# poke1024/vectorian

Hardware: AMD Instinct MI355X
Metric: sentence-alignments/sec at d=300, |q|=10, |s|<=64; 1/2/4/8 GPU + %HBM roofline (higher is better)
Workload: dtype bf16

## Files before the change

### vectorian_amd/csrc/vk_bound_host.h

```cpp
#ifndef VK_BOUND_HOST_H
#define VK_BOUND_HOST_H

#include "../../include/vectorian_hip.h"

#include <cmath>
#include <cstdint>
#include <cstring>
#include <vector>

#ifdef __HIPCC__
#define VK_HOST_DEVICE __host__ __device__
#define VK_UNROLL _Pragma("unroll")
#else
#define VK_HOST_DEVICE
#define VK_UNROLL
#endif

namespace vk_host {

struct shadow_format {
	int bits = 0;
	int d = 0;
	int steps = 0, step_features = 0;
	int live = 0, kept = 0;
// ... 132 lines not shown
		uint8_t *xq = codes.data();
		quant_meta m;
		if (fmt.bits == 8) { m = quantize_row_i8(x, d, reinterpret_cast<int8_t *>(xq)); i8_put_row(t.data(), i, xq, d); }
		else { m = quantize_row_e2m3(x, d, xq); fp6_put_row(t.data(), 4, i, xq, d); }
		bound_cell_constants(m, N, X, fmt.gamma_width, &cst[i], &cst[16 + i], &cst[32 + i]);
	}
	out.swap(t);
	return true;
}

struct bound_backoff {
	uint32_t recent = 0;
	int skip = 0;
	bool take() {
		if (skip > 0) { skip--; return false; }
		return true;
	}
	void record(bool fell_back) {
		recent = ((recent << 1) | (fell_back ? 1u : 0u)) & 0xffu;
		if (fell_back && __builtin_popcount(recent) >= 5) { skip = 64; recent = 0; }
	}
};

}

#endif
```

### vectorian_amd/csrc/vk_common.hip.h

```cpp

#ifndef VK_COMMON_HIP_H
#define VK_COMMON_HIP_H

#include <hip/hip_runtime.h>
#include <stdint.h>
#include <stdlib.h>

#include "vk_device.h"

typedef __attribute__((ext_vector_type(8))) short bf16x8;
typedef __attribute__((ext_vector_type(4))) short bf16x4;
typedef __attribute__((ext_vector_type(4))) float f32x4;
typedef __attribute__((ext_vector_type(4))) int i32x4;
typedef __attribute__((ext_vector_type(2))) float f32x2;

#define VK_NEG_INF (-__builtin_inff())
#define VK_RUN 4
#ifdef VK_DBG_NOINLINE
#define VK_DP_INLINE __attribute__((noinline))
#else
#define VK_DP_INLINE __forceinline__
#endif


// ... 186 lines not shown
	}
	return acc;
}
__device__ __forceinline__ f32x4 dot_tile_fp6(const uint8_t *__restrict__ qlds, const uint8_t *__restrict__ tile, int lane, int live6) {
	i32x4 lo[VK_DEV_FP6_STEPS];
	i32x2 hi[VK_DEV_FP6_STEPS];
	f32x2 meta;
	const uint32_t o16 = fp6_lane_offset(lane);
	load_tile_fp6<false>(lo, hi, meta, tile, lane, live6, o16);
	return mma_tile_fp6(lo, hi, qlds, o16);
}

__device__ __forceinline__ f32x4 cell_tile_fp6(const f32x4 acc, const f32x2 m, const uint8_t *__restrict__ qlds, int lane) {
	const float *cst = reinterpret_cast<const float *>(qlds + VK_DEV_FP6_QTILE_BYTES) + (lane >> 4) * 4;
	const f32x4 cs = *reinterpret_cast<const f32x4 *>(cst), ca = *reinterpret_cast<const f32x4 *>(cst + 16), cb = *reinterpret_cast<const f32x4 *>(cst + 32);
	f32x4 ub;
#pragma unroll
	for (int r = 0; r < 4; r++) ub[r] = clip01(((m[0] * cs[r]) * acc[r] + m[1] * ca[r]) + cb[r]);
	return ub;
}

#ifndef VK_FP6_TILES
#define VK_FP6_TILES 2
#endif
template <int T>
__device__ __forceinline__ void sim_tiles_fp6(f32x4 (&ub)[T], const uint8_t *__restrict__ qlds, const uint8_t *__restrict__ tile, int tile_bytes, int lane, int live6) {
	i32x4 lo[T][VK_DEV_FP6_STEPS];
	i32x2 hi[T][VK_DEV_FP6_STEPS];
	f32x2 meta[T];
	const uint32_t o16 = fp6_lane_offset(lane);
#pragma unroll
	for (int i = 0; i < T; i++) load_tile_fp6<true>(lo[i], hi[i], meta[i], tile + (int64_t)i * tile_bytes, lane, live6, o16);
	if constexpr (T > 1) __builtin_amdgcn_sched_barrier(0);
#pragma unroll
	for (int i = 0; i < T; i++) {
		ub[i] = cell_tile_fp6(mma_tile_fp6(lo[i], hi[i], qlds, o16), meta[i], qlds, lane);
		asm volatile("" : "+v"(ub[i]));
	}
}

template <int NB16>
__device__ __forceinline__ f32x4 sim_tile_f32_qlds(const uint8_t *__restrict__ qlds, const uint8_t *__restrict__ tile, int lane) {
	f32x4 x[NB16];
#pragma unroll
	for (int b = 0; b < NB16; b++) x[b] = __builtin_nontemporal_load(reinterpret_cast<const f32x4 *>(tile + b * 1024 + lane * 16));
	__builtin_amdgcn_sched_barrier(0);
// ... 503 lines not shown
			if (LT > 6) hc = fmaxf(hc, dpp_zero<0x116>(c) - wtv[6]);
			if (LT > 7) hc = fmaxf(hc, dpp_zero<0x117>(c) - wtv[7]);
			if (LT > 8) hc = fmaxf(hc, dpp_zero<0x118>(c) - wtv[8]);
			if (LT > 9) hc = fmaxf(hc, dpp_zero<0x119>(c) - wtv[9]);
			if (LT > 10) hc = fmaxf(hc, dpp_zero<0x11a>(c) - wtv[10]);
			if (LT > 11) hc = fmaxf(hc, dpp_zero<0x11b>(c) - wtv[11]);
			if (LT > 12) hc = fmaxf(hc, dpp_zero<0x11c>(c) - wtv[12]);
			if (LT > 13) hc = fmaxf(hc, dpp_zero<0x11d>(c) - wtv[13]);
			if (LT > 14) hc = fmaxf(hc, dpp_zero<0x11e>(c) - wtv[14]);
			if (LT > 15) hc = fmaxf(hc, dpp_zero<0x11f>(c) - wtv[15]);
			hreg[u] = hc;
			h = act ? hc : h;
			if (is_local || last_col) best = fmaxf(best, h);
		}
	}
	float m;
	if (is_local) m = v < a.len_t ? best : 0.0f;
	else if (is_global) m = last_col ? h : VK_NEG_INF;
	else m = v < a.len_t ? fmaxf(h, last_col ? best : 0.0f) : 0.0f;
	m = row_max_to_lane15(m);
	return (is_global) ? m : fmaxf(m, 0.0f);
}

template <int LT>
__device__ __forceinline__ float rwmd_rows(const float *__restrict__ S, int rowbase, int len, int maxlen, int v, const DpArgs &a) {
	const int len_t = a.len_t;
	const bool nbow = a.rwmd_normalize_bow != 0;
	const float w_t = nbow ? 1.0f / (float)len_t : 1.0f;
	const float w_s = nbow ? 1.0f / (float)(len > 0 ? len : 1) : 1.0f;
	const bool col_ok = v < len_t;
	float colmin = 3.402823466e+38F;
	float acc1 = 0.0f;
	for (int u = 1; u <= maxlen; u++) {
		const bool act = u <= len;
		const float s = S[(rowbase + (act ? u - 1 : 0)) * LT + v];
		const float dist = fmaxf(1.0f - s, 0.0f);
		if (act) colmin = fminf(colmin, dist);
		float m = col_ok ? dist : 3.402823466e+38F;
		m = fminf(m, dpp_f<DPP_ROW_SHR1>(m, m));
		m = fminf(m, dpp_f<DPP_ROW_SHR2>(m, m));
		m = fminf(m, dpp_f<DPP_ROW_SHR4>(m, m));
		m = fminf(m, dpp_f<DPP_ROW_SHR8>(m, m));
		if (act) acc1 += w_s * m;
	}
	const float x = col_ok ? w_t * colmin : 0.0f;
	float sum = x;
// ... 175 lines not shown
```

### vectorian_amd/csrc/vk_corpus.cpp

```cpp

#include "vk_internal.h"

std::string &vk_error_slot() {
	static thread_local std::string err;
	return err;
}

std::mutex &vk_ring_mutex() {
	static std::mutex mu;
	return mu;
}

void vk_devblock::release(void *p) {
	if (!p) return;
	{
		std::lock_guard<std::mutex> g(mu);
		ptrs.erase(std::remove(ptrs.begin(), ptrs.end(), p), ptrs.end());
	}
	(void)hipFree(p);
}

vk_devblock::~vk_devblock() {
	(void)hipSetDevice(device);
	for (void *p : ptrs) if (p) (void)hipFree(p);
// ... 540 lines not shown
int vk_bound_pass_state(vk_corpus_t *c, float *bounds, int64_t n, int64_t *counters) {
	if (!c || !counters) return fail(VK_ERR_INVALID, "null argument");
	const int64_t v[7] = {c->bp.ran, c->bp.round1, c->bp.round2, c->bp.fell_back, c->bp.queries, c->bp.fallbacks, c->bp.survivors};
	memcpy(counters, v, sizeof v);
	if (!bounds) return VK_OK;
	if (!c->bp.ran) return fail(VK_ERR_STATE, "the last query ran no bound pass");
	if (n != c->desc.n_sentences) return fail(VK_ERR_INVALID, "n differs from n_sentences");
	VK_HIP(hipSetDevice(c->device));
	std::vector<float> rows((size_t)c->n_entries);
	VK_HIP(hipMemcpy(rows.data(), c->d_ub, rows.size() * 4, hipMemcpyDeviceToHost));
	for (int64_t e = 0; e < c->n_entries; e++) {
		const int64_t sent = c->entry_sent.empty() ? e : (int64_t)c->entry_sent[(size_t)e];
		if (sent >= 0) bounds[sent] = rows[(size_t)e];
	}
	return VK_OK;
}

int vk_bound_pass_bits(vk_corpus_t *c, int64_t *bits) {
	if (!c || !bits) return fail(VK_ERR_INVALID, "null argument");
	*bits = c->shadow ? c->shadow_format.bits : 0;
	return VK_OK;
}

int vk_bound_pass_shadow(vk_corpus_t *c, int64_t *format, float *nx, int64_t tile0, int64_t n, uint8_t *out) {
	if (!c || !format || !nx) return fail(VK_ERR_INVALID, "null argument");
	const vk_host::shadow_format &sf = c->shadow_format;
	const int64_t f[5] = {sf.bits, sf.steps, sf.live, sf.tile_bytes(), c->n_tiles};
	memset(format, 0, sizeof f);
	nx[0] = nx[1] = 0.0f;
	if (!c->shadow) return out ? fail(VK_ERR_STATE, "the corpus has no shadow") : VK_OK;
	memcpy(format, f, sizeof f);
	nx[0] = c->shadow_n; nx[1] = c->shadow_x;
	if (!out) return VK_OK;
	if (tile0 < 0 || n < 0 || tile0 > c->n_tiles || n > c->n_tiles - tile0) return fail(VK_ERR_INVALID, "tiles out of range");
	VK_HIP(hipSetDevice(c->device));
	VK_HIP(hipStreamSynchronize(c->stream));
	if (n > 0) VK_HIP(hipMemcpy(out, c->shadow + tile0 * sf.tile_bytes(), (size_t)n * sf.tile_bytes(), hipMemcpyDeviceToHost));
	return VK_OK;
}

int vk_batch_state(vk_corpus_t *c, int64_t *state) {
	if (!c || !state) return fail(VK_ERR_INVALID, "null argument");
	memcpy(state, c->batch_state, sizeof c->batch_state);
	return VK_OK;
}

// ... 65 lines not shown
```

### vectorian_amd/csrc/vk_device.h

```cpp
#ifndef VK_DEVICE_H
#define VK_DEVICE_H

#include <hip/hip_runtime.h>
#include <stdint.h>

#define VK_DEV_LOCAL 0
#define VK_DEV_GLOBAL 1
#define VK_DEV_SEMIGLOBAL 2

#define VK_DEV_LAYOUT_CONTEXTUAL 0
#define VK_DEV_LAYOUT_STATIC 1

#define VK_DEV_MAX_SENT_LEN 64
#define VK_DEV_MAX_LONG_LEN 512
#define VK_DEV_MAX_QUERY_LEN 16
#define VK_DEV_MAX_WIDE_QUERY_LEN 64
#define VK_DEV_BOUND_CONST_BYTES 256
#define VK_DEV_FP6_STEPS 3
#define VK_DEV_FP6_STEP_BYTES 1536
#define VK_DEV_FP6_QTILE_BYTES (VK_DEV_FP6_STEPS * VK_DEV_FP6_STEP_BYTES)
#define VK_DEV_FP6_TILE_BYTES(live6) ((VK_DEV_FP6_STEPS - 1) * VK_DEV_FP6_STEP_BYTES + 384 * (live6) + 128)

struct VkScoreParams {
	const uint8_t *tiles;
	const int32_t *tok_id;
	const float *table;
	const int32_t *sent_start;
	const int32_t *sent_end;
	int32_t n_sent;
	int32_t layout;
	int32_t nk32, tail, tile_bytes;
	int32_t prec;
	int32_t q_lds;
	int32_t bound_bits;
	int32_t bound_live;
	int32_t q_mode3;
	const int32_t *group_list;
	int32_t n_list;
	int32_t max_short_len;
	const uint8_t *qtile;
	int32_t len_t;
	int32_t locality;
	int32_t gap_mode;
	int32_t rwmd_symmetric, rwmd_normalize_bow;
// ... 4 lines not shown
	const float *ws;
	const float *wt;
	const float *wt0;
	const float *boost;
	const int8_t *pos_s;
	const int8_t *tag_s;
	const uint32_t *qid_bits;
	int32_t slices_overlap;
	int32_t qkey[VK_DEV_MAX_QUERY_LEN];
	float tw[VK_DEV_MAX_QUERY_LEN];
	int32_t tpos[VK_DEV_MAX_QUERY_LEN];
	float tw_keep;
	float tw_threshold;
	float ref_total;
	const float *mag;
	float qmass[VK_DEV_MAX_QUERY_LEN];
	float wrd_raw_total;
	float *scores;
	float *raw;
	int32_t lds_floats_per_wave;
	int32_t s_rows_per_wave;
	int32_t h_rows;
	int32_t m_rows;
};

struct VkRwmdBatchParams {
	const uint8_t *tiles;
	int64_t n_tiles;
	int32_t tile_bytes, nk, half;
	const uint8_t *qtiles;
	int32_t n_qtiles, qpt;
	int32_t dense;
	int32_t late_mask;
	const int32_t *q_len;
	const float *q_inv_len;
	const float *q_param;
	int32_t n_queries;
	int32_t n_sent;
	int32_t tiles_per_sent;
	int32_t symmetric, nbow;
	const float *boost;
	float *scores;
	const int32_t *sent_len;
	const int32_t *sent_id;
	int64_t score_stride;
	const int32_t *tok_id;
// ... 236 lines not shown
hipError_t vk_launch_i8_probe(const int8_t *q, const int8_t *x, int32_t *out, hipStream_t stream);
hipError_t vk_launch_fp6_bound_probe(const uint8_t *qtile6, const uint8_t *tile6, int32_t live6, float *out, hipStream_t stream);
hipError_t vk_launch_select_ge_key(const float *scores, int64_t n, const uint64_t *theta_key, float floor_excl, uint64_t *keys_out,
	uint32_t *counter, uint32_t cap, hipStream_t stream);
hipError_t vk_launch_rekey(const uint64_t *keys, int32_t n, const float *scores, float floor_excl, uint64_t *out, hipStream_t stream);
hipError_t vk_launch_topk_unsorted(const uint64_t *in, int32_t n, int32_t k, uint64_t *out, hipStream_t stream);
hipError_t vk_launch_key_groups(const uint64_t *keys, int32_t n, int32_t *groups, hipStream_t stream);
hipError_t vk_launch_pack(const void *in, int32_t dtype_bf16, int64_t n_rows, int32_t d, int32_t d_pad, int64_t row0,
	uint8_t *tiles, float *mag_out, int32_t normalize, int32_t prec, hipStream_t stream);
size_t vk_score32_lds_bytes(int32_t nk32, int32_t tail, int32_t max_pair_tiles, int32_t len_t, int32_t gap_mode, int32_t waves);
int32_t vk_score32_waves(int32_t nk32, int32_t tail, int32_t max_pair_tiles, int32_t len_t, int32_t gap_mode);
hipError_t vk_launch_score32(const VkWideParams *p, int32_t max_pair_tiles, hipStream_t stream);
hipError_t vk_launch_filter_scan(const int8_t *pos, const int8_t *tag, uint64_t pos_mask, uint64_t tag_mask, int64_t n,
	int32_t *keep, int32_t *new_index, void *temp, size_t *temp_bytes, hipStream_t stream);
hipError_t vk_launch_filter_maps(const int32_t *keep, const int32_t *new_index, int64_t n, int32_t *src_of,
	const int32_t *start, const int32_t *end, int64_t n_entries, int32_t *out_start, int32_t *out_end, hipStream_t stream);
hipError_t vk_launch_filter_rows(const uint8_t *src, uint8_t *dst, const int32_t *src_of, int64_t n_kept, int32_t tile_bytes,
	hipStream_t stream);
hipError_t vk_launch_filter_gather(const void *src, void *dst, int32_t elem_bytes, const int32_t *src_of, int64_t n_kept,
	hipStream_t stream);
hipError_t vk_launch_table(const uint8_t *etiles, const uint8_t *qtile, int32_t n_tiles, int32_t nk32, int32_t tail,
	int32_t tile_bytes, float *table, const int32_t *q_ids, int32_t len_t, int32_t V, int32_t prec, hipStream_t stream);
hipError_t vk_launch_score(const VkScoreParams *p, int32_t grid, size_t smem_bytes, hipStream_t stream);
hipError_t vk_launch_span(const VkScoreParams *p, hipStream_t stream);
hipError_t vk_launch_score_batch(const VkScoreBatchParams *p, int32_t lt, size_t smem, hipStream_t stream);
hipError_t vk_launch_topk_scores(const float *scores, int64_t n, float min_score, int32_t k, uint64_t *out,
	int32_t *n_blocks_out, hipStream_t stream);
hipError_t vk_launch_topk_keys(const uint64_t *in, int64_t n, int32_t k, uint64_t *out, int32_t *n_blocks_out,
	hipStream_t stream);
hipError_t vk_launch_topk_wave(const float *scores, const uint64_t *keys_in, int64_t n, float min_score, int32_t k,
	int64_t per_wave, uint64_t *out, int64_t *n_waves_out, hipStream_t stream);
hipError_t vk_launch_flow(const VkFlowParams *p, int32_t k, hipStream_t stream);
hipError_t vk_launch_sort_all(const float *scores, int64_t n, float min_score, uint64_t *keys_a, uint64_t *keys_b, void *temp, size_t *temp_bytes,
	uint64_t **sorted_out, hipStream_t stream);
hipError_t vk_launch_rwmd_batch(const VkRwmdBatchParams *p, hipStream_t stream);
hipError_t vk_launch_rwmd_batch32(const VkRwmdBatchParams *p, hipStream_t stream);
hipError_t vk_launch_batch_pack(const uint8_t *src_tiles, uint8_t *dst_tiles, const int32_t *ids, const int32_t *sent_start, const int32_t *sent_end,
	int64_t n, int32_t tps, int32_t tile_bytes, hipStream_t stream);
int vk_rwmd_batch_supported(int32_t nk, int32_t half);
hipError_t vk_launch_table_batch(const uint8_t *etiles, int64_t n_vtiles, int32_t tile_bytes, int32_t nk16, const uint8_t *qtiles, int32_t n_qtiles,
	uint16_t *table, hipStream_t stream);
hipError_t vk_launch_table_batch_fix(uint16_t *table, const int64_t *offsets, int32_t n, hipStream_t stream);
hipError_t vk_launch_rwmd_static32(const VkRwmdBatchParams *p, int32_t w64, hipStream_t stream);
hipError_t vk_launch_topk_wave_batch(const float *scores, const uint64_t *keys_in, int64_t n, float min_score, int32_t k,
	int64_t per_wave, int32_t n_queries, int64_t in_stride, int64_t out_stride, uint64_t *out, int64_t *n_waves_out, hipStream_t stream);
hipError_t vk_launch_wrd_exact(const VkWrdParams *p, int32_t n_cand, float *scores_to_mark, hipStream_t stream);
// ... 13 lines not shown
```

### vectorian_amd/csrc/vk_internal.h

```cpp
#ifndef VK_INTERNAL_H
#define VK_INTERNAL_H

#include "../../include/vectorian_hip.h"
#include "vk_device.h"
#include "vk_devbuf.h"
#include "vk_guard.h"
#include "vk_result_host.h"
#include "vk_bound_host.h"
#include "vk_route_host.h"

#include <algorithm>
#include <atomic>
#include <cmath>
#include <cstdio>
#include <cstring>
#include <memory>
#include <mutex>
#include <string>
#include <vector>

std::string &vk_error_slot();

namespace {

// ... 24 lines not shown
	uint32_t u = ((uint32_t)b) << 16;
	float f;
	memcpy(&f, &u, 4);
	return f;
}

using vk_host::gap_cost;

constexpr int kTopkChunk = 2048;
constexpr int kGapTable = 640;
constexpr int64_t kStageBytes = 64ll << 20;
constexpr int64_t kBoundPassMinSentences = 1000000;
constexpr int64_t kBoundRound2Floor = 1024;
inline int bound_pass_mode() {
	const char *e = getenv("VK_BOUND_PASS");
	return !e ? 0 : !strcmp(e, "off") ? -1 : !strcmp(e, "force") ? 1 : 0;
}
inline int bound_bits_wanted(int mode) {
	const char *e = getenv("VK_BOUND_BITS");
	if (e && !strcmp(e, "6")) return 6;
	if (e && !strcmp(e, "8")) return 8;
	return mode > 0 ? 8 : 6;
}

}

struct vk_devblock {
	int device = 0;
	std::mutex mu;
	std::vector<void *> ptrs;
	void add(void *p) { std::lock_guard<std::mutex> g(mu); ptrs.push_back(p); }
	void release(void *p);
	~vk_devblock();
};

std::mutex &vk_ring_mutex();

struct vk_corpus_shape {
	vk_corpus_desc desc{};
	int device = 0;
	int d_pad = 0, nk32 = 0, tail = 0, tile_bytes = 0;
	int prec = 0;
	int64_t rows_total = 0, rows_appended = 0, n_tiles = 0;
	uint8_t *d_tiles = nullptr;
	float *d_mag = nullptr;
	int32_t *d_tok_id = nullptr;
// ... 54 lines not shown
	vk_devbuf<float> d_out_raw, d_out_sim;
	vk_devbuf<int16_t> d_out_map;
	vk_devbuf<float> d_wrd_raw, d_wrd_val;
	vk_devbuf<uint32_t> d_counter;
	vk_devbuf<float> d_rows_out, d_plan_out;
	vk_devbuf<uint8_t> d_bqt; vk_devbuf<uint64_t> d_bcand; vk_devbuf<int32_t> d_bcandq; vk_devbuf<float> d_brows;
	vk_devbuf<float, true> h_brows;
	vk_devbuf<uint32_t> d_qbits;
	vk_devbuf<uint8_t> d_wrdl_scratch;
	vk_devbuf<uint8_t> d_wide_scratch;
	vk_devbuf<int32_t> d_apart_order; int32_t n_apart_order = -1;
	vk_devbuf<int32_t> d_xlong_order; int32_t n_xlong_order = -1;
	vk_devbuf<int32_t> d_wide_order; int32_t n_wide_order = -1;
	int rows_w = 0;
	struct batch_bucket { vk_devbuf<uint8_t> tiles; vk_devbuf<int32_t> len, id; int64_t n = 0; };
	batch_bucket bl[4];
	bool bl_built = false;
	int64_t bl_empty = 0;
	vk_devbuf<uint8_t> d_qtile8; vk_devbuf<float> d_ub; vk_devbuf<int32_t> d_bound_groups; vk_devbuf<uint64_t> d_bound_keys;
	struct bound_state {
		bool pruned = false;
		VkScoreParams full{}; int full_grid = 0; size_t full_smem = 0;
		int64_t ran = 0, round1 = 0, round2 = 0, fell_back = 0;
		int64_t queries = 0, fallbacks = 0, survivors = 0;
		vk_host::bound_backoff backoff;
	} bp;
	vk_devbuf<int32_t> d_sb_id[2]; int64_t sb_n[2] = {0, 0}; bool sb_built = false; int64_t sb_empty = 0;
	vk_devbuf<uint16_t> d_btable;
	vk_devbuf<int64_t> d_bfix;
	vk_devbuf<int32_t> d_bqids;
	vk_devbuf<uint64_t> d_sort[2]; vk_devbuf<uint8_t> d_sort_temp;
	int64_t batch_state[VK_BS_COUNT] = {};
	int64_t query_route[VK_QR_COUNT] = {};
	hipEvent_t ev[7] = {nullptr, nullptr, nullptr, nullptr, nullptr, nullptr, nullptr};
	vk_timings last{};
	bool have_scores = false;
	bool is_view = false;
	struct longq_bufs {
		vk_devbuf<uint8_t> qt;
		vk_devbuf<float> fl;
		vk_devbuf<int32_t> il;
		vk_devbuf<float> table;
		vk_devbuf<uint8_t> scratch, fscratch;
		vk_devbuf<uint8_t> bscratch;
		vk_devbuf<int32_t> order; int32_t n_order = -1;
		vk_devbuf<float> raw, sim;
// ... 132 lines not shown
```

### vectorian_amd/csrc/vk_query.cpp

```cpp

#include "vk_internal.h"
#include "vk_guard.h"
#include "vk_transport_host.h"

static constexpr int kCanonMargin = 8;
static const vk_host::route_fits kRouteFits{vk_score32_waves, vk_wide_ring_rows, vk_wide_lds_demand};
static bool exact_transport(const vk_query_desc *q) { return vk_host::exact_transport(q->algorithm, q->wmd_full != 0); }
static vk_host::route_facts route_facts_of(const vk_corpus *c, const vk_query_desc *q, const vk_topk_out *out) {
	vk_host::route_facts f;
	f.layout = c->desc.layout; f.prec = c->prec; f.nk32 = c->nk32; f.tail = c->tail;
	f.max_len = c->max_len; f.max_short_len = c->max_short_len; f.n_long_groups = c->n_long_groups;
	f.has_apart = c->h_apart && !c->h_apart->empty(); f.has_xlong = c->h_xlong && !c->h_xlong->empty();
	f.max_pair_tiles = c->max_pair_tiles; f.max_short_pair_tiles = c->max_short_pair_tiles; f.uniform_len = c->uniform_len;
	f.has_pos = c->d_pos != nullptr; f.has_tags = c->d_tag != nullptr; f.n_sentences = c->desc.n_sentences;
	f.algorithm = q->algorithm; f.wmd_full = q->wmd_full != 0; f.rwmd_injective = q->rwmd_injective != 0; f.len_t = q->len_t;
	if (q->algorithm == VK_ALG_ALIGN) {
		f.gaps = vk_host::classify_gaps(q->gap_s, q->gap_t);
		if (f.gaps.gap_mode == 2 && q->gap_s.kind >= VK_GAP_LINEAR && q->gap_s.kind <= VK_GAP_TABLE) f.ws_tail = vk_host::ws_tail_of(q->gap_s, c->max_len);
	}
	f.submatch = q->submatch_weight > 0.0f; f.tagged = q->tag_weights != nullptr; f.has_q_tags = q->q_tags != nullptr; f.has_q_ids = q->q_token_ids != nullptr;
	f.only = q->only_slices != nullptr; f.want_flow = q->want_flow != 0; f.locality = q->locality;
	f.sim_rows = out->sim_rows != nullptr; f.raw_score = out->raw_score != nullptr; f.boost = q->boost != nullptr;
	const int k = q->max_matches;
	const bool restated = (q->want_flow && q->algorithm == VK_ALG_ALIGN) || (q->algorithm == VK_ALG_RWMD && !q->wmd_full && q->want_flow && out->sim_rows);
// ... 119 lines not shown
			if (c->prec) {
				const size_t off = (size_t)(i >> 4) * c->tile_bytes + (size_t)(k >> 4) * 1024 + (size_t)((k & 3) * 16 + (i & 15)) * 16 + (size_t)((k & 15) >> 2) * 4;
				memcpy(&tile[off], &row[(size_t)k], 4);
				continue;
			}
			const uint16_t b = f32_to_bf16(row[(size_t)k]);
			const int t = k >> 5, g = (k & 31) >> 3, j = k & 7;
			const size_t off = (size_t)(i >> 4) * c->tile_bytes + (size_t)t * 1024 + (size_t)(g * 16 + (i & 15)) * 16 + (size_t)j * 2;
			memcpy(&tile[off], &b, 2);
		}
	}
	if (!bound_tile || !c->shadow || c->prec || q->len_t > VK_FAST_QUERY_LEN) return;
	std::vector<float> stored((size_t)q->len_t * d);
	for (int i = 0; i < q->len_t; i++)
		for (int k = 0; k < d; k++) {
			uint16_t b;
			memcpy(&b, &tile[(size_t)(k >> 5) * 1024 + (size_t)(((k & 31) >> 3) * 16 + i) * 16 + (size_t)(k & 7) * 2], 2);
			stored[(size_t)i * d + k] = bf16_to_f32(b);
		}
	vk_host::pack_bound_query(c->shadow_format, stored.data(), q->len_t, c->shadow_n, c->shadow_x, *bound_tile);
}

static int score_bounded(vk_corpus *c, const VkScoreParams &p, int grid, size_t smem, size_t smem_bound, size_t smem_list, int kk, float sel_floor,
	vk_host_keep &keep, hipStream_t st, const uint64_t **d_sel) {
	*d_sel = nullptr;
	const int64_t n = c->n_entries;
	vk_corpus::bound_state &b = c->bp;
	const int64_t most = std::max<int64_t>(n / 16, kBoundRound2Floor);
	const int M = kk <= 32 ? 64 : kk <= 256 ? 512 : VK_MAX_MATCHES;
	int rc;
	if ((rc = c->d_ub.reserve((size_t)n + 8, &c->device_bytes))) return rc;
	if ((rc = c->d_bound_groups.reserve((size_t)std::max<int64_t>(most, kTopkChunk), &c->device_bytes))) return rc;
	if ((rc = c->d_bound_keys.reserve((size_t)2 * kTopkChunk, &c->device_bytes))) return rc;
	if ((rc = c->d_counter.reserve(4, &c->device_bytes))) return rc;
	VkScoreParams pb = p;
	const vk_host::shadow_format &sf = c->shadow_format;
	pb.tiles = c->shadow; pb.nk32 = sf.steps; pb.tail = 0; pb.tile_bytes = sf.tile_bytes(); pb.bound_bits = sf.bits; pb.bound_live = sf.live;
	pb.q_mode3 = 0; pb.q_lds = 0; pb.qtile = c->d_qtile8; pb.scores = c->d_ub; pb.raw = nullptr;
	VK_HIP(vk_launch_score(&pb, grid, smem_bound, st));
	VK_HIP(hipEventRecord(c->ev[2], st));
	c->ev2_recorded = true;
	b.ran = 1; b.queries++;
	VK_HIP(hipMemsetD32Async(static_cast<hipDeviceptr_t>(c->d_scores), (int)0xff800000u, (size_t)n, st));
	if (p.raw) VK_HIP(hipMemsetD32Async(reinterpret_cast<hipDeviceptr_t>(p.raw), (int)0xff800000u, (size_t)n, st));
	VkScoreParams pl = p;
	pl.group_list = c->d_bound_groups;
	const uint64_t *d_first = nullptr;
	if ((rc = select_blocks(c, sel_floor, M, st, &d_first, c->d_ub))) return rc;
	VK_HIP(vk_launch_key_groups(d_first, M, c->d_bound_groups, st));
	pl.n_list = M;
	VK_HIP(vk_launch_score(&pl, M, smem_list, st));
	uint64_t *d_exact = c->d_bound_keys, *d_best = c->d_bound_keys + kTopkChunk;
	VK_HIP(vk_launch_rekey(d_first, M, c->d_scores, sel_floor, d_exact, st));
	VK_HIP(vk_launch_topk_unsorted(d_exact, M, kk, d_best, st));
	VK_HIP(vk_launch_select_ge_key(c->d_ub, n, d_best + (kk - 1), sel_floor, c->d_keys[0], c->d_counter, (uint32_t)most, st));
	uint32_t &count = *keep.array<uint32_t>(1);
	VK_HIP(hipMemcpyAsync(&count, c->d_counter, 4, hipMemcpyDeviceToHost, st));
	VK_HIP(hipStreamSynchronize(st));
	b.round1 = M;
	bool fell = false;
	if ((int64_t)count > most) {
// ... 2 lines not shown
	} else if (count > 0) {
		VK_HIP(vk_launch_key_groups(c->d_keys[0], (int32_t)count, c->d_bound_groups, st));
		pl.n_list = (int32_t)count;
		VK_HIP(vk_launch_score(&pl, (int32_t)count, smem_list, st));
	}
	if (!fell && count <= (uint32_t)kTopkChunk) {
		VK_HIP(vk_launch_rekey(c->d_keys[0], (int32_t)count, c->d_scores, sel_floor, d_exact, st));
		VK_HIP(vk_launch_topk_unsorted(d_exact, (int32_t)count, kk, d_best, st));
		*d_sel = d_best;
	}
	b.round2 = count;
	if (!fell) b.survivors += count;
	b.fell_back = fell ? 1 : 0;
	if (fell) b.fallbacks++;
	if (bound_pass_mode() == 0) b.backoff.record(fell);
	b.pruned = !fell;
	b.full = p; b.full_grid = grid; b.full_smem = smem;
	return VK_OK;
}

static int query_body(vk_corpus_t *c, const vk_query_desc *q, vk_topk_out *out, vk_host_keep &keep) {
	int rc = VK_OK;
	VK_HIP(hipSetDevice(c->device));
	c->bp.pruned = false; c->bp.ran = c->bp.round1 = c->bp.round2 = c->bp.fell_back = 0;
	for (int64_t &x : c->query_route) x = -1;
	if (q->len_t > VK_MAX_QUERY_LEN) return vk_longq_query(c, q, out, keep);
	hipStream_t st = c->stream;
	const int64_t n = c->n_entries;
	const int k = q->max_matches;
	const bool only = q->only_slices != nullptr;
	out->n_out = 0;
	c->have_scores = false;
	if (n == 0) return VK_OK;
	const vk_host::route_switches sw = vk_host::read_route_switches();
	vk_host::route_facts facts = route_facts_of(c, q, out);
	const int bound_mode = bound_pass_mode();
	facts.bound_pass = c->shadow && bound_mode >= 0 && (bound_mode > 0 || c->desc.n_sentences >= kBoundPassMinSentences) && vk_host::bound_pass_takes(facts) &&
		(bound_mode != 0 || c->bp.backoff.take());
	const vk_host::query_route r = vk_host::route_query(facts, sw, kRouteFits);
	if (r.status != VK_OK) return fail(r.status, r.message);
	const int64_t route_state[VK_QR_COUNT] = {r.plan, r.gap_mode, r.wide_gap_mode, r.score32_gap_mode, r.wave_tiles, r.pass[vk_host::CLASS_SHORT],
		r.pass[vk_host::CLASS_MID], r.pass[vk_host::CLASS_XLONG], r.list, r.ring_rows, r.flow, r.ostride, r.raw, r.span_skip_raw};
	memcpy(c->query_route, route_state, sizeof route_state);
	const bool wide_query = q->len_t > VK_FAST_QUERY_LEN;
	const bool xlong = c->max_len > VK_MAX_SENT_LEN;
	const bool wide_family = r.flow != vk_host::FLOW_NARROW;
	auto sentence_of = [c](int64_t row) { return c->entry_sent.empty() ? row : (int64_t)c->entry_sent[(size_t)row]; };
// ... 267 lines not shown
	p.m_rows = (c->max_short_len + 4) / 4 * 4;
	if (p.gap_mode == 7) lds_floats += 4 * p.m_rows;
	p.lds_floats_per_wave = lds_floats;
	size_t smem = (size_t)lds_floats * 4 * 4;
	const bool reg_history = p.gap_mode == 3 || p.gap_mode == 6;
	if (!is_static && c->prec == 0 && c->nk32 == 10 && c->tail == 1)
		p.q_mode3 = sw.qlds ? 1 : sw.qreg ? 0 : (reg_history ? 1 : 0);
	if (!is_static && c->prec == 1 && c->nk32 == 19 && !sw.no_f32_special) p.q_mode3 = 1;
	const size_t qlds = (!is_static && ((c->prec == 0 && c->nk32 == 24 && c->tail == 0) || p.q_mode3)) ? (size_t)c->nk32 * 1024 : 0;
	smem += qlds;
	if (!is_static && qlds == 0 && !(c->prec == 0 && c->nk32 == 10 && c->tail == 1)) {
		const size_t qb = ((size_t)c->tile_bytes + 1023) / 1024 * 1024;
		if (2 * (smem + qb) <= 160 * 1024 && !sw.no_qlds1) { p.q_lds = (int32_t)qb; smem += qb; }
	}
	if (smem > 160 * 1024) return fail(VK_ERR_UNSUPPORTED, "LDS demand exceeds 160 KiB per workgroup");
	const int64_t n_groups = (n + 3) / 4;
	const int grid = (int)std::min<int64_t>((n_groups + 3) / 4, (int64_t)1 << 20);
	bounded = bound_ok;
	if (!bounded && r.plan == vk_host::PLAN_BOUNDED) c->query_route[VK_QR_PLAN] = vk_host::PLAN_FUSED;
	if (bounded) {
		const size_t smem_strips = smem - qlds - (size_t)p.q_lds;
		const size_t smem_bound = smem_strips + (size_t)c->shadow_format.qtile_bytes() + VK_DEV_BOUND_CONST_BYTES;
		const size_t smem_list = (size_t)lds_floats * 4 + qlds + (size_t)p.q_lds;
		if ((rc = score_bounded(c, p, grid, smem, smem_bound, smem_list, kk, sel_floor, keep, st, &d_sel_bounded))) return rc;
	} else if (r.plan != vk_host::PLAN_LISTED) VK_HIP(vk_launch_score(&p, grid, smem, st));
	if (r.pass[vk_host::CLASS_MID] == vk_host::PASS_FUSED_LONG) {
		VkScoreParams pl = p;
		pl.group_list = c->d_long_groups; pl.n_list = c->n_long_groups;
		if (pl.gap_mode == 3 || pl.gap_mode == 6) pl.gap_mode = 2;
		pl.s_rows_per_wave = is_static ? (c->long_group_tokens + 15) / 16 * 16 : c->long_group_tiles * 16;
		pl.h_rows = 0;
		int lf = pl.s_rows_per_wave * lt + 16;
		if (pl.gap_mode == 2) lf += (c->max_long_len + 1) * 16;
		pl.m_rows = 0;
		if (pl.gap_mode == 7) lf += (c->max_long_len + 4) / 4 * 4;
		pl.lds_floats_per_wave = lf;
		const size_t smem_l = (size_t)lf * 4 + qlds + (size_t)pl.q_lds;
		if (smem_l > 160 * 1024) return fail(VK_ERR_UNSUPPORTED, "LDS demand of the long-slice pass exceeds 160 KiB");
		VK_HIP(vk_launch_score(&pl, c->n_long_groups, smem_l, st));
	}
	if (r.wide_pass != vk_host::PASS_NONE && (rc = list_pass())) return rc;
	}

	if (exact_transport(q) && only) {
		const int cnt = q->n_only;
		std::vector<uint64_t> &hk = keep.vec<uint64_t>((size_t)cnt);
		std::vector<int64_t> rows_idx((size_t)cnt);
// ... 461 lines not shown
```

### vectorian_amd/csrc/vk_score.hip.h

```cpp
#ifndef VK_SCORE_HIP_H
#define VK_SCORE_HIP_H

#include <type_traits>
#include "vk_common.hip.h"


#ifdef VK_SCORE_VGPRS
#define VK_SCORE_KERNEL_ATTR __attribute__((amdgpu_num_vgpr(VK_SCORE_VGPRS)))
#else
#define VK_SCORE_KERNEL_ATTR
#endif

template <int MODE, int NK32, bool TAIL, int GAP, int LT>
__global__ __launch_bounds__(256) VK_SCORE_KERNEL_ATTR void vk_score_kernel(VkScoreParams p) {
	extern __shared__ float4 vk_smem4[];
	float *smem = reinterpret_cast<float *>(vk_smem4);
	const int lane = threadIdx.x & 63, wv = threadIdx.x >> 6;
	const int nwaves = blockDim.x >> 6;
	const uint8_t *qlds = reinterpret_cast<const uint8_t *>(smem);
	if constexpr (MODE == 3 || MODE == 4) {
		for (int i = threadIdx.x; i < NK32 * 64; i += blockDim.x)
			vk_smem4[i] = *reinterpret_cast<const float4 *>(p.qtile + i * 16);
		__syncthreads();
		smem += NK32 * 256;
// ... 21 lines not shown
	float *S = smem + wv * p.lds_floats_per_wave;
	float *Hh = S + p.s_rows_per_wave * LT + 16;
	const int sigma = lane >> 4, v = lane & 15;

	QFrag<NK32, TAIL> qf;
	if constexpr (MODE == 0) load_qfrag<NK32, TAIL>(qf, p.qtile, lane);

	DpArgs a;
	a.locality = p.locality; a.len_t = p.len_t;
	a.gs = p.gs; a.gt = p.gt; a.a_s = p.a_s; a.a_t = p.a_t; a.open_s = p.open_s; a.open_t = p.open_t;
	a.ws = p.ws; a.wt = p.wt; a.wt0 = p.wt0;
	a.rwmd_symmetric = p.rwmd_symmetric; a.rwmd_normalize_bow = p.rwmd_normalize_bow; a.wmd_bound = p.wmd_bound;
	a.wrd_raw_total = p.wrd_raw_total;
	const float inv_ref = p.ref_total;
	constexpr bool TAGS = MODE != 7 && MODE != 8;
	float twl[4] = {1.0f, 1.0f, 1.0f, 1.0f};
	int tposl[4] = {0, 0, 0, 0};
	if (TAGS && p.pos_s) {
		const int cbase = (MODE == 2) ? (lane & 3) * 4 : (lane >> 4) * 4;
#pragma unroll
		for (int r = 0; r < 4; r++) { twl[r] = p.tw[cbase + r]; tposl[r] = p.tpos[cbase + r]; }
	}

	constexpr int WSN = GAP == 6 ? 65 : 33;
	float wsr[WSN], wtr[LT];
	if (GAP == 3 || GAP == 6) {
#pragma unroll
		for (int k = 0; k < WSN; k++) wsr[k] = p.ws[k];
#pragma unroll
		for (int k = 0; k < LT; k++) wtr[k] = p.wt[k];
	}

	const int n_groups = p.group_list ? p.n_list : (p.n_sent + 3) >> 2;
	const int run = p.group_list ? 1 : VK_RUN;
	const int n_runs = (n_groups + run - 1) / run;
	for (int ri = blockIdx.x * nwaves + wv; ri < n_runs; ri += gridDim.x * nwaves) {
	int prev_tile = -1, prev_row = 0;
	for (int gg = 0; gg < run; gg++) {
		const int gi = ri * run + gg;
		if (gi >= n_groups) break;
		const int grp = p.group_list ? p.group_list[gi] : gi;
		const int s_idx = grp * 4 + sigma;
		const int i0 = s_idx < p.n_sent ? s_idx : p.n_sent;
		const int t_a = p.sent_start[i0], t_b = p.sent_end[i0];
		const int len = t_b - t_a;
		const int g_a = __builtin_amdgcn_readlane(t_a, 0);
		const int g_b = __builtin_amdgcn_readlane(t_b, 48);
		int maxlen = __builtin_amdgcn_readlane(len, 0);
		maxlen = max(maxlen, __builtin_amdgcn_readlane(len, 16));
		maxlen = max(maxlen, __builtin_amdgcn_readlane(len, 32));
		maxlen = max(maxlen, __builtin_amdgcn_readlane(len, 48));
// ... 27 lines not shown
						}
						if ((lane & 3) * 4 < LT) *reinterpret_cast<float4 *>(S + tk * LT + (lane & 3) * 4) = vq;
					}
				}
			}
			rowbase = t_a - g_a;
		} else {
			const int tile0 = g_a >> 4;
			const int ntiles = ((g_b + 15) >> 4) - tile0;
			const uint8_t *tp = p.tiles + (int64_t)tile0 * p.tile_bytes;
			int ti0 = 0;
			if (ntiles > 0 && tile0 == prev_tile) {
				if (prev_row != 0) {
					float4 keep = {0.0f, 0.0f, 0.0f, 0.0f};
					if (lane < 4 * LT) keep = reinterpret_cast<const float4 *>(S)[prev_row * 4 * LT + lane];
					wave_lds_fence();
					if (lane < 4 * LT) reinterpret_cast<float4 *>(S)[lane] = keep;
				}
				ti0 = 1;
				tp += p.tile_bytes;
			}
			if (ntiles > 0) { prev_tile = tile0 + ntiles - 1; prev_row = ntiles - 1; }
			if constexpr (MODE == 8) {
				constexpr int T = GAP == 6 ? 1 : VK_FP6_TILES;
				const auto tiles = [&](auto tc, int ti) {
					constexpr int N = decltype(tc)::value;
					f32x4 ub[N];
					sim_tiles_fp6<N>(ub, qlds, tp, p.tile_bytes, lane, p.bound_live);
#pragma unroll
					for (int i = 0; i < N; i++)
						if ((lane >> 4) * 4 < LT) *reinterpret_cast<f32x4 *>(S + ((ti + i) * 16 + (lane & 15)) * LT + (lane >> 4) * 4) = ub[i];
					tp += (int64_t)N * p.tile_bytes;
				};
				int ti = ti0;
				for (; ti + T <= ntiles; ti += T) tiles(std::integral_constant<int, T>{}, ti);
				if constexpr (T > 1)
					for (; ti < ntiles; ti++) tiles(std::integral_constant<int, 1>{}, ti);
			} else
			for (int ti = ti0; ti < ntiles; ti++) {
				f32x4 acc;
				if constexpr (MODE == 0) acc = sim_tile<NK32, TAIL>(qf, tp, lane);
				else if constexpr (MODE == 3) acc = sim_tile_qlds<NK32, TAIL>(qlds, tp, lane);
				else if constexpr (MODE == 4) acc = sim_tile_f32_qlds<NK32>(qlds, tp, lane);
				else if constexpr (MODE == 7) acc = sim_tile_i8<NK32>(qlds, tp, lane, p.bound_live);
				else {
					constexpr bool DEEP = MODE == 5 || MODE == 6;
					constexpr int PREC = MODE == 6 ? 1 : 0;
// ... 12 lines not shown
		}
		wave_lds_fence();
		int turns = 1;
		bool rewrite = false;
		if constexpr (MODE == 2 && (GAP == 4 || GAP == 7)) {
			if (p.qid_bits) {
				rewrite = len > 0 && static_vocab_shared(len, p.len_t, p.tok_id + t_a, p.tag_s + t_a, p.qid_bits, p.qkey) != 0;
				if (p.slices_overlap && __builtin_amdgcn_ballot_w64(rewrite) != 0) turns = 4;
				else if (rewrite) static_vocab_fixup<16>(S + rowbase * LT, LT, len, p.len_t, p.tok_id + t_a, p.tag_s + t_a, p.pos_s + t_a, p.table, 0,
					p.qid_bits, p.qkey, p.tw, p.tpos, p.tw_keep, p.tw_threshold, v);
				wave_lds_fence();
			}
		}

		const int lenc = len > 0 ? len : 0;
		const int rb = len > 0 ? rowbase : 0;
		auto evaluate = [&]() -> float {
		float raw;
		if constexpr (GAP == 0) raw = dp_linear<LT>(S, rb, lenc, maxlen, v, a);
		else if constexpr (GAP == 1) raw = dp_affine<LT>(S, rb, lenc, maxlen, v, a);
		else if constexpr (GAP == 2) raw = dp_general<LT>(S, Hh, p.h_rows, rb, lenc, maxlen, lane, a);
		else if constexpr (GAP == 3) raw = dp_general_reg<LT, 32>(S, rb, lenc, maxlen, v, a, wsr, wtr);
		else if constexpr (GAP == 6) raw = dp_general_reg<LT, 64, MODE != 7>(S, rb, lenc, maxlen, v, a, wsr, wtr);
		else if constexpr (GAP == 4) {
			if (a.wmd_bound == 1) raw = wrd_bound_rows<LT>(S, rb, lenc, maxlen, v, a, nullptr, nullptr, 1.0f / (float)a.len_t);
			else raw = rwmd_rows<LT>(S, rb, lenc, maxlen, v, a);
		}
		else if constexpr (GAP == 7) {
			float *sm = nullptr;
			if (MODE == 2) {
				sm = Hh + sigma * p.m_rows;
				const float wsum = p.rwmd_normalize_bow ? (float)(lenc > 0 ? lenc : 1) : 1.0f;
				for (int u = v; u < lenc; u += 16) {
					const int id = p.tok_id[t_a + u];
					int cnt = 0;
					bool first = true;
					for (int i = 0; i < lenc; i++) {
						const bool same = p.tok_id[t_a + i] == id && (!p.tag_s || p.tag_s[t_a + i] == p.tag_s[t_a + u]);
						cnt += same ? 1 : 0;
						first = first && !(same && i < u);
					}
					sm[u] = first ? (float)cnt / wsum : 0.0f;
				}
				wave_lds_fence();
			}
			raw = rwmd_fill_rows<LT>(S, sm, rb, lenc, maxlen, lane, a, p.qmass[v]);
// ... 92 lines not shown
```

### vectorian_amd/csrc/vk_score_m7.hip

```cpp
#define VK_SCORE_VGPRS 120
#include "vk_score.hip.h"

extern "C" hipError_t vk_launch_score_m7w(const VkScoreParams *p, int32_t grid, size_t smem_bytes, hipStream_t stream);
template <int NK64>
static hipError_t launch_m7(const VkScoreParams *p, int32_t grid, size_t smem_bytes, hipStream_t stream) {
	switch (p->gap_mode) {
	case 0: return launch_score_lt<7, NK64, false, 0>(*p, grid, smem_bytes, stream);
	case 1: return launch_score_lt<7, NK64, false, 1>(*p, grid, smem_bytes, stream);
	case 3: return launch_score_lt<7, NK64, false, 3>(*p, grid, smem_bytes, stream);
	case 6: return vk_launch_score_m7w(p, grid, smem_bytes, stream);
	default: return hipErrorInvalidValue;
	}
}
extern "C" hipError_t vk_launch_score_m7(const VkScoreParams *p, int32_t grid, size_t smem_bytes, hipStream_t stream) {
	if (p->bound_live < 1 || p->bound_live > 4) return hipErrorInvalidValue;
	if (p->pos_s) return hipErrorInvalidValue;
	if (p->nk32 == 5) return launch_m7<5>(p, grid, smem_bytes, stream);
	if (p->nk32 == 12) return launch_m7<12>(p, grid, smem_bytes, stream);
	return hipErrorInvalidValue;
}
```

### vectorian_amd/csrc/vk_score_m8.hip

```cpp
#define VK_SCORE_VGPRS 120
#include "vk_score.hip.h"

extern "C" hipError_t vk_launch_score_m8w(const VkScoreParams *p, int32_t grid, size_t smem_bytes, hipStream_t stream);
extern "C" hipError_t vk_launch_score_m8(const VkScoreParams *p, int32_t grid, size_t smem_bytes, hipStream_t stream) {
	if (p->bound_live < 1 || p->bound_live > 4 || p->tile_bytes != VK_DEV_FP6_TILE_BYTES(p->bound_live)) return hipErrorInvalidValue;
	if (p->pos_s) return hipErrorInvalidValue;
	switch (p->gap_mode) {
	case 0: return launch_score_lt<8, VK_DEV_FP6_STEPS, false, 0>(*p, grid, smem_bytes, stream);
	case 1: return launch_score_lt<8, VK_DEV_FP6_STEPS, false, 1>(*p, grid, smem_bytes, stream);
	case 3: return launch_score_lt<8, VK_DEV_FP6_STEPS, false, 3>(*p, grid, smem_bytes, stream);
	case 6: return vk_launch_score_m8w(p, grid, smem_bytes, stream);
	default: return hipErrorInvalidValue;
	}
}
```

Before: 720.8 million.

## Use flat-tailed gap table in bound pass to cut DP inner loop cost

Adds a bound-pass DP variant (gap modes 8/9) that keeps only the first K gap costs exactly and replaces all longer gaps with the minimum tail cost, tracked through a running max. This turns the O(K_max) inner gap loop of the general-gap DP into O(K) plus a single update. Because the cost is never larger than the true one, the result is still an upper bound. It also lowers the VGPR budget for the new fp6 kernel and makes the variant the default when bound_mode is 0, with an env override. The looser bound may let more candidates through pruning into the full scoring pass.

```diff
diff --git a/vectorian_amd/csrc/vk_bound_host.h b/vectorian_amd/csrc/vk_bound_host.h
--- a/vectorian_amd/csrc/vk_bound_host.h
+++ b/vectorian_amd/csrc/vk_bound_host.h
@@ -178,6 +178,17 @@
 	}
 };
 
+inline float bound_tail_cost(const float *w, int k, int rows) {
+	float c = INFINITY;
+	for (int j = k + 1; j <= rows; j++) c = w[j] < c ? w[j] : c;
+	return c;
+}
+inline bool bound_tail_choice(const char *env, int mode) {
+	if (env && !strcmp(env, "0")) return false;
+	if (env && !strcmp(env, "1")) return true;
+	return mode == 0;
+}
+
 }
 
 #endif
diff --git a/vectorian_amd/csrc/vk_common.hip.h b/vectorian_amd/csrc/vk_common.hip.h
--- a/vectorian_amd/csrc/vk_common.hip.h
+++ b/vectorian_amd/csrc/vk_common.hip.h
@@ -232,6 +232,12 @@
 
 #ifndef VK_FP6_TILES
 #define VK_FP6_TILES 2
+#endif
+#ifndef VK_FP6_TILES_TAIL
+#define VK_FP6_TILES_TAIL 2
+#endif
+#ifndef VK_FP6_TILES_TAIL64
+#define VK_FP6_TILES_TAIL64 1
 #endif
 template <int T>
 __device__ __forceinline__ void sim_tiles_fp6(f32x4 (&ub)[T], const uint8_t *__restrict__ qlds, const uint8_t *__restrict__ tile, int tile_bytes, int lane, int live6) {
@@ -781,6 +787,77 @@
 	return (is_global) ? m : fmaxf(m, 0.0f);
 }
 
+template <int LT, int MAXLEN, int KT, bool FRESH = true>
+__device__ __forceinline__ float dp_general_tail_reg(const float *__restrict__ S, int rowbase, int len, int maxlen, int v,
+	const DpArgs &a, const float (&wsr)[KT + 2], const float (&wtr)[LT]) {
+	static_assert(KT >= 1 && KT < MAXLEN, "the tail begins inside the table");
+	int loc = a.locality, vsel = v;
+	if constexpr (FRESH) {
+		asm volatile("" : "+v"(loc));
+		asm volatile("" : "+v"(vsel));
+		loc = __builtin_amdgcn_readfirstlane(loc);
+	}
+	const bool is_local = loc == VK_DEV_LOCAL;
+	const bool is_global = loc == VK_DEV_GLOBAL;
+	const float floor0 = is_local ? 0.0f : VK_NEG_INF;
+	const bool last_col = v == a.len_t - 1;
+	const float wt_border = a.wt[v + 1];
+	const float wt_border0 = a.wt0[v + 1];
+	const float c_tail = wsr[KT + 1];
+
+	float wtv[16];
+#pragma unroll
+	for (int k = 1; k < LT; k++) wtv[k] = vsel >= k ? wtr[k] : __builtin_inff();
+
+	float hreg[MAXLEN + 1];
+	float h = is_global ? -wt_border0 : 0.0f;
+	hreg[0] = h;
+	float R = h;
+	float best = 0.0f;
+#pragma unroll
+	for (int u = 1; u <= MAXLEN; u++) {
+		if (u <= maxlen) {
+			const bool act = u <= len;
+			const float s = S[(rowbase + (act ? u - 1 : 0)) * LT + v];
+			const float bprev = is_global ? -wsr[u - 1 <= KT ? u - 1 : KT + 1] : 0.0f;
+			const float bcur = is_global ? -wsr[u <= KT ? u : KT + 1] : 0.0f;
+			const float diag = dpp_f<DPP_ROW_SHR1>(bprev, hreg[u - 1]);
+			float c = fmaxf(diag + s, floor0);
+#pragma unroll
+			for (int k = 1; k <= (u < KT ? u : KT); k++) c = fmaxf(c, hreg[u - k] - wsr[k]);
+			if (u > KT) {
+				if (u > KT + 1) R = fmaxf(R, hreg[u - KT - 1]);
+				c = fmaxf(c, R - c_tail);
+			}
+			float hc = fmaxf(c, bcur - wt_border);
+			if (LT > 1) hc = fmaxf(hc, dpp_zero<0x111>(c) - wtv[1]);
+			if (LT > 2) hc = fmaxf(hc, dpp_zero<0x112>(c) - wtv[2]);
+			if (LT > 3) hc = fmaxf(hc, dpp_zero<0x113>(c) - wtv[3]);
+			if (LT > 4) hc = fmaxf(hc, dpp_zero<0x114>(c) - wtv[4]);
+			if (LT > 5) hc = fmaxf(hc, dpp_zero<0x115>(c) - wtv[5]);
+			if (LT > 6) hc = fmaxf(hc, dpp_zero<0x116>(c) - wtv[6]);
+			if (LT > 7) hc = fmaxf(hc, dpp_zero<0x117>(c) - wtv[7]);
+			if (LT > 8) hc = fmaxf(hc, dpp_zero<0x118>(c) - wtv[8]);
+			if (LT > 9) hc = fmaxf(hc, dpp_zero<0x119>(c) - wtv[9]);
+			if (LT > 10) hc = fmaxf(hc, dpp_zero<0x11a>(c) - wtv[10]);
+			if (LT > 11) hc = fmaxf(hc, dpp_zero<0x11b>(c) - wtv[11]);
+			if (LT > 12) hc = fmaxf(hc, dpp_zero<0x11c>(c) - wtv[12]);
+			if (LT > 13) hc = fmaxf(hc, dpp_zero<0x11d>(c) - wtv[13]);
+			if (LT > 14) hc = fmaxf(hc, dpp_zero<0x11e>(c) - wtv[14]);
+			if (LT > 15) hc = fmaxf(hc, dpp_zero<0x11f>(c) - wtv[15]);
+			hreg[u] = hc;
+			h = act ? hc : h;
+			if (is_local || last_col) best = fmaxf(best, h);
+		}
+	}
+	float m;
+	if (is_local) m = v < a.len_t ? best : 0.0f;
+	else if (is_global) m = last_col ? h : VK_NEG_INF;
+	else m = v < a.len_t ? fmaxf(h, last_col ? best : 0.0f) : 0.0f;
+	m = row_max_to_lane15(m);
+	return (is_global) ? m : fmaxf(m, 0.0f);
+}
+
 template <int LT>
 __device__ __forceinline__ float rwmd_rows(const float *__restrict__ S, int rowbase, int len, int maxlen, int v, const DpArgs &a) {
 	const int len_t = a.len_t;
diff --git a/vectorian_amd/csrc/vk_corpus.cpp b/vectorian_amd/csrc/vk_corpus.cpp
--- a/vectorian_amd/csrc/vk_corpus.cpp
+++ b/vectorian_amd/csrc/vk_corpus.cpp
@@ -586,6 +586,12 @@
 	return VK_OK;
 }
 
+int vk_bound_pass_tail(vk_corpus_t *c, int32_t *k) {
+	if (!c || !k) return fail(VK_ERR_INVALID, "null argument");
+	*k = c->bp.ran ? (int32_t)c->bp.tail_k : 0;
+	return VK_OK;
+}
+
 int vk_bound_pass_shadow(vk_corpus_t *c, int64_t *format, float *nx, int64_t tile0, int64_t n, uint8_t *out) {
 	if (!c || !format || !nx) return fail(VK_ERR_INVALID, "null argument");
 	const vk_host::shadow_format &sf = c->shadow_format;
diff --git a/vectorian_amd/csrc/vk_device.h b/vectorian_amd/csrc/vk_device.h
--- a/vectorian_amd/csrc/vk_device.h
+++ b/vectorian_amd/csrc/vk_device.h
@@ -20,6 +20,10 @@
 #define VK_DEV_FP6_STEP_BYTES 1536
 #define VK_DEV_FP6_QTILE_BYTES (VK_DEV_FP6_STEPS * VK_DEV_FP6_STEP_BYTES)
 #define VK_DEV_FP6_TILE_BYTES(live6) ((VK_DEV_FP6_STEPS - 1) * VK_DEV_FP6_STEP_BYTES + 384 * (live6) + 128)
+
+#ifndef VK_BOUND_TAIL_K
+#define VK_BOUND_TAIL_K 4
+#endif
 
 struct VkScoreParams {
 	const uint8_t *tiles;
@@ -70,6 +74,7 @@
 	int32_t s_rows_per_wave;
 	int32_t h_rows;
 	int32_t m_rows;
+	float bound_tail_cost;
 };
 
 struct VkRwmdBatchParams {
@@ -352,6 +357,8 @@
 hipError_t vk_launch_table(const uint8_t *etiles, const uint8_t *qtile, int32_t n_tiles, int32_t nk32, int32_t tail,
 	int32_t tile_bytes, float *table, const int32_t *q_ids, int32_t len_t, int32_t V, int32_t prec, hipStream_t stream);
 hipError_t vk_launch_score(const VkScoreParams *p, int32_t grid, size_t smem_bytes, hipStream_t stream);
+int32_t vk_score_m8t_tail_k(void);
+int32_t vk_score_m7t_tail_k(void);
 hipError_t vk_launch_span(const VkScoreParams *p, hipStream_t stream);
 hipError_t vk_launch_score_batch(const VkScoreBatchParams *p, int32_t lt, size_t smem, hipStream_t stream);
 hipError_t vk_launch_topk_scores(const float *scores, int64_t n, float min_score, int32_t k, uint64_t *out,
diff --git a/vectorian_amd/csrc/vk_internal.h b/vectorian_amd/csrc/vk_internal.h
--- a/vectorian_amd/csrc/vk_internal.h
+++ b/vectorian_amd/csrc/vk_internal.h
@@ -70,6 +70,7 @@
 	if (e && !strcmp(e, "8")) return 8;
 	return mode > 0 ? 8 : 6;
 }
+inline bool bound_tail_wanted(int mode) { return vk_host::bound_tail_choice(getenv("VK_BOUND_TAIL"), mode); }
 
 }
 
@@ -170,6 +171,7 @@
 		bool pruned = false;
 		VkScoreParams full{}; int full_grid = 0; size_t full_smem = 0;
 		int64_t ran = 0, round1 = 0, round2 = 0, fell_back = 0;
+		int64_t tail_k = 0;
 		int64_t queries = 0, fallbacks = 0, survivors = 0;
 		vk_host::bound_backoff backoff;
 	} bp;
diff --git a/vectorian_amd/csrc/vk_query.cpp b/vectorian_amd/csrc/vk_query.cpp
--- a/vectorian_amd/csrc/vk_query.cpp
+++ b/vectorian_amd/csrc/vk_query.cpp
@@ -165,7 +165,7 @@
 }
 
 static int score_bounded(vk_corpus *c, const VkScoreParams &p, int grid, size_t smem, size_t smem_bound, size_t smem_list, int kk, float sel_floor,
-	vk_host_keep &keep, hipStream_t st, const uint64_t **d_sel) {
+	const vk_gap &gap_s, bool tail, vk_host_keep &keep, hipStream_t st, const uint64_t **d_sel) {
 	*d_sel = nullptr;
 	const int64_t n = c->n_entries;
 	vk_corpus::bound_state &b = c->bp;
@@ -180,6 +180,15 @@
 	const vk_host::shadow_format &sf = c->shadow_format;
 	pb.tiles = c->shadow; pb.nk32 = sf.steps; pb.tail = 0; pb.tile_bytes = sf.tile_bytes(); pb.bound_bits = sf.bits; pb.bound_live = sf.live;
 	pb.q_mode3 = 0; pb.q_lds = 0; pb.qtile = c->d_qtile8; pb.scores = c->d_ub; pb.raw = nullptr;
+	b.tail_k = 0;
+	if (tail && (p.gap_mode == 3 || p.gap_mode == 6)) {
+		const int rows = p.gap_mode == 3 ? 32 : 64, K = sf.bits == 6 ? vk_score_m8t_tail_k() : vk_score_m7t_tail_k();
+		float w[65];
+		for (int j = 0; j <= rows; j++) w[j] = gap_cost(gap_s, j);
+		pb.gap_mode = p.gap_mode == 3 ? 8 : 9;
+		pb.bound_tail_cost = vk_host::bound_tail_cost(w, K, rows);
+		b.tail_k = K;
+	}
 	VK_HIP(vk_launch_score(&pb, grid, smem_bound, st));
 	VK_HIP(hipEventRecord(c->ev[2], st));
 	c->ev2_recorded = true;
@@ -228,7 +237,7 @@
 static int query_body(vk_corpus_t *c, const vk_query_desc *q, vk_topk_out *out, vk_host_keep &keep) {
 	int rc = VK_OK;
 	VK_HIP(hipSetDevice(c->device));
-	c->bp.pruned = false; c->bp.ran = c->bp.round1 = c->bp.round2 = c->bp.fell_back = 0;
+	c->bp.pruned = false; c->bp.ran = c->bp.round1 = c->bp.round2 = c->bp.fell_back = c->bp.tail_k = 0;
 	for (int64_t &x : c->query_route) x = -1;
 	if (q->len_t > VK_MAX_QUERY_LEN) return vk_longq_query(c, q, out, keep);
 	hipStream_t st = c->stream;
@@ -542,7 +551,7 @@
 		const size_t smem_strips = smem - qlds - (size_t)p.q_lds;
 		const size_t smem_bound = smem_strips + (size_t)c->shadow_format.qtile_bytes() + VK_DEV_BOUND_CONST_BYTES;
 		const size_t smem_list = (size_t)lds_floats * 4 + qlds + (size_t)p.q_lds;
-		if ((rc = score_bounded(c, p, grid, smem, smem_bound, smem_list, kk, sel_floor, keep, st, &d_sel_bounded))) return rc;
+		if ((rc = score_bounded(c, p, grid, smem, smem_bound, smem_list, kk, sel_floor, q->gap_s, bound_tail_wanted(bound_mode), keep, st, &d_sel_bounded))) return rc;
 	} else if (r.plan != vk_host::PLAN_LISTED) VK_HIP(vk_launch_score(&p, grid, smem, st));
 	if (r.pass[vk_host::CLASS_MID] == vk_host::PASS_FUSED_LONG) {
 		VkScoreParams pl = p;
diff --git a/vectorian_amd/csrc/vk_score.hip.h b/vectorian_amd/csrc/vk_score.hip.h
--- a/vectorian_amd/csrc/vk_score.hip.h
+++ b/vectorian_amd/csrc/vk_score.hip.h
@@ -67,11 +67,14 @@
 		for (int r = 0; r < 4; r++) { twl[r] = p.tw[cbase + r]; tposl[r] = p.tpos[cbase + r]; }
 	}
 
-	constexpr int WSN = GAP == 6 ? 65 : 33;
+	constexpr bool FLAT = GAP == 8 || GAP == 9;
+	static_assert(!FLAT || MODE == 7 || MODE == 8, "a flat-tailed table gives a bound, not a score");
+	constexpr int WSN = FLAT ? VK_BOUND_TAIL_K + 2 : GAP == 6 ? 65 : 33;
 	float wsr[WSN], wtr[LT];
-	if (GAP == 3 || GAP == 6) {
-#pragma unroll
-		for (int k = 0; k < WSN; k++) wsr[k] = p.ws[k];
+	if (GAP == 3 || GAP == 6 || FLAT) {
+#pragma unroll
+		for (int k = 0; k < (FLAT ? WSN - 1 : WSN); k++) wsr[k] = p.ws[k];
+		if (FLAT) wsr[WSN - 1] = p.bound_tail_cost;
 #pragma unroll
 		for (int k = 0; k < LT; k++) wtr[k] = p.wt[k];
 	}
@@ -145,7 +148,7 @@
 			}
 			if (ntiles > 0) { prev_tile = tile0 + ntiles - 1; prev_row = ntiles - 1; }
 			if constexpr (MODE == 8) {
-				constexpr int T = GAP == 6 ? 1 : VK_FP6_TILES;
+				constexpr int T = GAP == 6 ? 1 : GAP == 8 ? VK_FP6_TILES_TAIL : GAP == 9 ? VK_FP6_TILES_TAIL64 : VK_FP6_TILES;
 				const auto tiles = [&](auto tc, int ti) {
 					constexpr int N = decltype(tc)::value;
 					f32x4 ub[N];
@@ -204,6 +207,8 @@
 		else if constexpr (GAP == 2) raw = dp_general<LT>(S, Hh, p.h_rows, rb, lenc, maxlen, lane, a);
 		else if constexpr (GAP == 3) raw = dp_general_reg<LT, 32>(S, rb, lenc, maxlen, v, a, wsr, wtr);
 		else if constexpr (GAP == 6) raw = dp_general_reg<LT, 64, MODE != 7>(S, rb, lenc, maxlen, v, a, wsr, wtr);
+		else if constexpr (GAP == 8) raw = dp_general_tail_reg<LT, 32, VK_BOUND_TAIL_K>(S, rb, lenc, maxlen, v, a, wsr, wtr);
+		else if constexpr (GAP == 9) raw = dp_general_tail_reg<LT, 64, VK_BOUND_TAIL_K, MODE != 7>(S, rb, lenc, maxlen, v, a, wsr, wtr);
 		else if constexpr (GAP == 4) {
 			if (a.wmd_bound == 1) raw = wrd_bound_rows<LT>(S, rb, lenc, maxlen, v, a, nullptr, nullptr, 1.0f / (float)a.len_t);
 			else raw = rwmd_rows<LT>(S, rb, lenc, maxlen, v, a);
diff --git a/vectorian_amd/csrc/vk_score_m7.hip b/vectorian_amd/csrc/vk_score_m7.hip
--- a/vectorian_amd/csrc/vk_score_m7.hip
+++ b/vectorian_amd/csrc/vk_score_m7.hip
@@ -2,6 +2,7 @@
 #include "vk_score.hip.h"
 
 extern "C" hipError_t vk_launch_score_m7w(const VkScoreParams *p, int32_t grid, size_t smem_bytes, hipStream_t stream);
+extern "C" hipError_t vk_launch_score_m7t(const VkScoreParams *p, int32_t grid, size_t smem_bytes, hipStream_t stream);
 template <int NK64>
 static hipError_t launch_m7(const VkScoreParams *p, int32_t grid, size_t smem_bytes, hipStream_t stream) {
 	switch (p->gap_mode) {
@@ -15,6 +16,7 @@
 extern "C" hipError_t vk_launch_score_m7(const VkScoreParams *p, int32_t grid, size_t smem_bytes, hipStream_t stream) {
 	if (p->bound_live < 1 || p->bound_live > 4) return hipErrorInvalidValue;
 	if (p->pos_s) return hipErrorInvalidValue;
+	if (p->gap_mode == 8 || p->gap_mode == 9) return vk_launch_score_m7t(p, grid, smem_bytes, stream);
 	if (p->nk32 == 5) return launch_m7<5>(p, grid, smem_bytes, stream);
 	if (p->nk32 == 12) return launch_m7<12>(p, grid, smem_bytes, stream);
 	return hipErrorInvalidValue;
diff --git a/vectorian_amd/csrc/vk_score_m7t.hip b/vectorian_amd/csrc/vk_score_m7t.hip
--- /dev/null
+++ b/vectorian_amd/csrc/vk_score_m7t.hip
@@ -0,0 +1,17 @@
+#include "vk_score.hip.h"
+
+extern "C" int32_t vk_score_m7t_tail_k(void) { return VK_BOUND_TAIL_K; }
+
+template <int NK64>
+static hipError_t launch_m7t(const VkScoreParams *p, int32_t grid, size_t smem_bytes, hipStream_t stream) {
+	switch (p->gap_mode) {
+	case 8: return launch_score_lt<7, NK64, false, 8>(*p, grid, smem_bytes, stream);
+	case 9: return launch_score_lt<7, NK64, false, 9>(*p, grid, smem_bytes, stream);
+	default: return hipErrorInvalidValue;
+	}
+}
+extern "C" hipError_t vk_launch_score_m7t(const VkScoreParams *p, int32_t grid, size_t smem_bytes, hipStream_t stream) {
+	if (p->nk32 == 5) return launch_m7t<5>(p, grid, smem_bytes, stream);
+	if (p->nk32 == 12) return launch_m7t<12>(p, grid, smem_bytes, stream);
+	return hipErrorInvalidValue;
+}
diff --git a/vectorian_amd/csrc/vk_score_m8.hip b/vectorian_amd/csrc/vk_score_m8.hip
--- a/vectorian_amd/csrc/vk_score_m8.hip
+++ b/vectorian_amd/csrc/vk_score_m8.hip
@@ -2,6 +2,7 @@
 #include "vk_score.hip.h"
 
 extern "C" hipError_t vk_launch_score_m8w(const VkScoreParams *p, int32_t grid, size_t smem_bytes, hipStream_t stream);
+extern "C" hipError_t vk_launch_score_m8t(const VkScoreParams *p, int32_t grid, size_t smem_bytes, hipStream_t stream);
 extern "C" hipError_t vk_launch_score_m8(const VkScoreParams *p, int32_t grid, size_t smem_bytes, hipStream_t stream) {
 	if (p->bound_live < 1 || p->bound_live > 4 || p->tile_bytes != VK_DEV_FP6_TILE_BYTES(p->bound_live)) return hipErrorInvalidValue;
 	if (p->pos_s) return hipErrorInvalidValue;
@@ -10,6 +11,7 @@
 	case 1: return launch_score_lt<8, VK_DEV_FP6_STEPS, false, 1>(*p, grid, smem_bytes, stream);
 	case 3: return launch_score_lt<8, VK_DEV_FP6_STEPS, false, 3>(*p, grid, smem_bytes, stream);
 	case 6: return vk_launch_score_m8w(p, grid, smem_bytes, stream);
+	case 8: case 9: return vk_launch_score_m8t(p, grid, smem_bytes, stream);
 	default: return hipErrorInvalidValue;
 	}
 }
diff --git a/vectorian_amd/csrc/vk_score_m8t.hip b/vectorian_amd/csrc/vk_score_m8t.hip
--- /dev/null
+++ b/vectorian_amd/csrc/vk_score_m8t.hip
@@ -0,0 +1,12 @@
+#define VK_SCORE_VGPRS 104
+#include "vk_score.hip.h"
+
+extern "C" int32_t vk_score_m8t_tail_k(void) { return VK_BOUND_TAIL_K; }
+
+extern "C" hipError_t vk_launch_score_m8t(const VkScoreParams *p, int32_t grid, size_t smem_bytes, hipStream_t stream) {
+	switch (p->gap_mode) {
+	case 8: return launch_score_lt<8, VK_DEV_FP6_STEPS, false, 8>(*p, grid, smem_bytes, stream);
+	case 9: return launch_score_lt<8, VK_DEV_FP6_STEPS, false, 9>(*p, grid, smem_bytes, stream);
+	default: return hipErrorInvalidValue;
+	}
+}
```

Measured after the change: 784.4 million, median of 6. +8.8%, better.
